# tensorflow/adanet

Hardware: NVIDIA H100
Metric: candidate-train examples/sec per AdaNet iteration (higher is better)
Workload: dtype f32

## Files before the change

### adanet_b200/_lib.py

```python

from __future__ import annotations

import ctypes
import os
from ctypes import POINTER, c_char_p, c_float, c_int, c_int64, c_void_p

_HERE = os.path.dirname(os.path.abspath(__file__))
LIB_PATH = os.path.join(_HERE, "csrc", "libadanet_b200.so")

ACT_NONE, ACT_RELU = 0, 1
HEAD_SOFTMAX_XENT, HEAD_MSE, HEAD_SIGMOID_XENT = 0, 1, 2
MIX_SCALAR, MIX_VECTOR, MIX_MATRIX = 0, 1, 2
OPT_SGD, OPT_MOMENTUM, OPT_RMSPROP, OPT_ADAM, OPT_MOMENTUM_COSINE = 0, 1, 2, 3, 4
PATH_AUTO, PATH_SIMT, PATH_TCGEN05 = 0, 1, 2
PLANES_TF32, PLANES_F16 = 0, 1
(Q_VERSION, Q_DENSE_BWD_WS, Q_HEAD_WS, Q_DENSE_FWD_PATH, Q_SM_COUNT, Q_LAUNCH_COUNT, Q_DENSE_BWD_PATH,
 Q_DENSE_FWD_WS, Q_PLANES_BYTES, Q_DENSE_BWD_P_WS, Q_COLSUM_WS, Q_CONV_STEM_BWD_WS, Q_PLANE_FORMAT,
 Q_TMA_MAP_CACHE_HITS, Q_TMA_MAP_CACHE_MISSES) = range(15)

EXPORTS = (
    "adn_last_error", "adn_init", "adn_query", "adn_set_dense_path", "adn_dense_fwd", "adn_dense_bwd", "adn_head_loss",
    "adn_ensemble_head", "adn_opt_step", "adn_l1_norm", "adn_ema_update", "adn_record_scalars",
    "adn_counter_add", "adn_planes_split", "adn_planes_merge", "adn_dense_fwd_p", "adn_dense_bwd_p", "adn_colsum",
    "adn_opt_step_p", "adn_head_loss_p", "adn_dense_fwd_p_group", "adn_dense_bwd_p_group",
    "adn_l1_grad_add", "adn_conv_stem_fwd", "adn_conv_stem_bwd", "adn_set_plane_format", "adn_plane_overflow",
    "adn_planes_split_scaled", "adn_head_group", "adn_head_bookkeeping", "adn_opt_step_group",
)


class FwdOp(ctypes.Structure):
  _fields_ = [("xp", c_void_p), ("wp", c_void_p), ("bias", c_void_p), ("yp", c_void_p), ("y", c_void_p),
              ("in_", c_int64), ("out", c_int64), ("act", ctypes.c_int32), ("reserved", ctypes.c_int32),
              ("dropout_rate", c_float), ("dropout_seed", ctypes.c_uint32), ("dropout_layer", ctypes.c_int32),
              ("reserved2", ctypes.c_int32), ("dropout_step_dev", c_void_p)]


class BwdOp(ctypes.Structure):
  _fields_ = [("xp", c_void_p), ("wp", c_void_p), ("dzp", c_void_p), ("dxp", c_void_p), ("dx", c_void_p),
              ("dx_colsum", c_void_p), ("dw", c_void_p), ("in_", c_int64), ("out", c_int64),
              ("x_relu_mask", ctypes.c_int32), ("dz_log2_scale", ctypes.c_int32), ("workspace", c_void_p),
              ("workspace_bytes", c_int64), ("dx_mul", c_float), ("reserved2", c_float)]


class HeadOp(ctypes.Structure):
  _fields_ = [("head", ctypes.c_int32), ("mixture_type", ctypes.c_int32), ("members_host", POINTER(c_void_p)),
              ("n_members", ctypes.c_int32), ("reg_is_zero", ctypes.c_int32), ("w", c_void_p), ("bias", c_void_p),
              ("gammas_host", POINTER(c_float)), ("reg_multiplier", c_float), ("dz_log2_scale", ctypes.c_int32),
              ("labels", c_void_p), ("labels_f", c_void_p), ("out3", c_void_p), ("dw", c_void_p), ("dbias", c_void_p),
              ("dens", c_void_p), ("ens_out", c_void_p), ("dens_planes", c_void_p), ("colsum_only", ctypes.c_int32),
# ... 128 lines not shown
```

### adanet_b200/core/engine.py

```python

from __future__ import annotations

import ctypes
import math
from dataclasses import dataclass, field
from typing import Dict, List, Optional, Sequence, Tuple

import numpy as np
import torch

from adanet_b200 import _lib

_HEAD_KIND = {"softmax_xent": _lib.HEAD_SOFTMAX_XENT, "mse": _lib.HEAD_MSE, "sigmoid_xent": _lib.HEAD_SIGMOID_XENT}
_MIX_KIND = {"scalar": _lib.MIX_SCALAR, "vector": _lib.MIX_VECTOR, "matrix": _lib.MIX_MATRIX}
_OPT_KIND = {"sgd": _lib.OPT_SGD, "momentum": _lib.OPT_MOMENTUM, "rmsprop": _lib.OPT_RMSPROP, "adam": _lib.OPT_ADAM,
             "momentum_cosine": _lib.OPT_MOMENTUM_COSINE}
_OPT_DEFAULTS = {"sgd": (), "momentum": (), "rmsprop": (0.9, 0.0, 1e-10), "adam": (0.9, 0.999, 1e-8),
                 "momentum_cosine": (0.0,)}
TRACE_FIELDS = ("sub_loss", "ens_loss", "adanet_loss", "ema")
EVAL_METRICS = ("adanet_loss", "loss", "average_loss", "accuracy")


def accuracy_of(logits: torch.Tensor, labels: torch.Tensor) -> float:
  if logits.shape[1] > 1:
# ... 215 lines not shown
      self.stem_k = torch.as_tensor(k).to(device)
      self.stem_b = torch.as_tensor(np.ascontiguousarray(bs[0], dtype=np.float32)).to(device)
      self.stem_out = new_planes(batch, dims[0], device)
      self.stem_arg = torch.zeros((batch * dims[0] // 16,), dtype=torch.int32, device=device)
      ws, bs = ws[1:], bs[1:]
    self.in_dim = int(np.prod(self.image_shape)) if self.stem else self.dims[0]
    self.fmt = _lib.plane_format()
    assert len(ws) == len(dims) - 1
    self.ws = [torch.as_tensor(np.ascontiguousarray(w, dtype=np.float32)).to(device) for w in ws]
    self.bs = [torch.as_tensor(np.ascontiguousarray(b, dtype=np.float32)).to(device) for b in bs]
    for i, w in enumerate(self.ws):
      if tuple(w.shape) != (dims[i], dims[i + 1]):
        raise ValueError("kernel %d of %s has shape %s, want %s" % (i, name, tuple(w.shape), (dims[i], dims[i + 1])))
    self.planes = planes_enabled()
    n = len(self.ws)
    if self.planes:
      self.acts = [None] * (n - 1) + [torch.empty((batch, dims[-1]), dtype=torch.float32, device=device)]
      self.hp = [new_planes(batch, d, device) for d in dims[1:-1]]
      self.wps = [new_planes(dims[i], dims[i + 1], device) for i in range(n)]
      self.refresh_planes()
      self.fwd_ws_bytes, self.fwd_ws = 0, None
    else:
      self.acts = [torch.empty((batch, d), dtype=torch.float32, device=device) for d in dims[1:]]
      self.hp, self.wps = None, None
      fwd_ws = max(_lib.query(_lib.Q_DENSE_FWD_WS, batch, dims[i], dims[i + 1]) for i in range(n))
      self.fwd_ws_bytes = fwd_ws
      self.fwd_ws = torch.empty((max(fwd_ws, 16),), dtype=torch.uint8, device=device)

  def ensure_format(self):
    if not self.planes or self.fmt == _lib.plane_format():
      return
    self.fmt = _lib.plane_format()
    n = len(self.ws)
    self.hp = [new_planes(self.batch, d, self.device) for d in self.dims[1:-1]]
    self.wps = [new_planes(self.dims[i], self.dims[i + 1], self.device) for i in range(n)]
    if self.stem:
# ... 37 lines not shown
    out = torch.empty((self.batch, self.dims[-2]), dtype=torch.float32, device=self.device)
    _lib.check(_lib.load().adn_planes_merge(self.hp[-1].data_ptr(), self.batch, self.dims[-2], out.data_ptr(),
                                            torch.cuda.current_stream(self.device).cuda_stream), "adn_planes_merge")
    return out

  def fwd_op(self, i: int, xp: torch.Tensor, step_dev: Optional[torch.Tensor] = None) -> "_lib.FwdOp":
    last = i == len(self.ws) - 1
    src = (self.stem_out if self.stem else xp) if i == 0 else self.hp[i - 1]
    op = _lib.FwdOp(src.data_ptr(), self.wps[i].data_ptr(), self.bs[i].data_ptr(),
                    None if last else self.hp[i].data_ptr(), self.acts[i].data_ptr() if last else None,
                    self.dims[i], self.dims[i + 1], _lib.ACT_NONE if last else _lib.ACT_RELU, 0)
    d = self.dropout[i] if (self.dropout and step_dev is not None and not last and i < len(self.dropout)) else None
    if d is not None:
      op.dropout_rate, op.dropout_seed, op.dropout_layer = float(d[0]), int(d[1]) & 0xffffffff, i
      op.dropout_step_dev = step_dev.data_ptr()
    return op

  def dx_mul(self, i: int) -> float:
    d = self.dropout[i] if (self.dropout and 0 <= i < len(self.dropout)) else None
    return 1.0 / (1.0 - float(d[0])) if d is not None else 1.0

  def forward(self, lib, x: torch.Tensor, sp: int, xp: Optional[torch.Tensor] = None):
    n = len(self.ws)
    if self.planes:
      hp = xp
      if self.stem:
        self.stem_forward(lib, x, sp)
        hp = self.stem_out
      for i in range(n):
        last = i == n - 1
# ... 555 lines not shown
    st["pending"] = False

  def _enqueue_waves(self):
    lib = self.lib
    main = torch.cuda.current_stream(self.device)
    sp = main.cuda_stream
    bag = [c for c in self.candidates if c.bagged]
    if bag:
      for c in bag:
        if c.xp_own is not None:
          _lib.check(lib.adn_planes_split(c.x_own.data_ptr(), self.batch, c.net.in_dim, c.xp_own.data_ptr(), sp),
                     "adn_planes_split")
        else:
          c.net.stem_forward(lib, c.x_own, sp)
      for w in range(max(len(c.net.ws) for c in bag)):
        ops = [c.net.fwd_op(w, c.xp_own, self.step_dev) for c in bag if w < len(c.net.ws)]
        _lib.check(lib.adn_dense_fwd_p_group((_lib.FwdOp * len(ops))(*ops), len(ops), self.batch, sp),
                   "adn_dense_fwd_p_group")
      for c in bag:
        lab_i = c.labels_own if self.labels is not None else None
        lab_f = c.labels_own if self.labels is None else None
        c.enqueue_sub_loss(lab_i, lab_f, sp, loss_out=c.own_loss)
      for k in range(max(len(c.net.ws) for c in bag)):
        ops = [c.bwd_op(k, c.xp_own) for c in bag if k < len(c.net.ws)]
        _lib.check(lib.adn_dense_bwd_p_group((_lib.BwdOp * len(ops))(*ops), len(ops), self.batch, sp),
                   "adn_dense_bwd_p_group")
      for c in bag:
        if c.net.stem:
          c.enqueue_stem_bwd(c.x_own, sp)
        c.enqueue_sub_update(sp)
    self._split_x(sp)
# ... 1 lines not shown
      if c.xp_local is not None:
        _lib.check(lib.adn_planes_split(self.x.data_ptr() + c.row0 * self.in_dim * 4, c.batch, self.in_dim,
                                        c.xp_local.data_ptr(), sp), "adn_planes_split")
    xp_of = lambda c: c.xp_local if c.xp_local is not None else self.xp
    x_of = lambda c: self.x[c.row0:c.row0 + c.batch] if c.comm is not None else self.x
    for f in self.frozen:
      if f.stem:
        f.stem_forward(lib, self.x, sp)
    for c in self.candidates:
      if c.net.stem:
        c.net.stem_forward(lib, x_of(c), sp)
    fwd = ([(f, self.xp, self.batch, None) for f in self.frozen] +
           [(c.net, xp_of(c), c.batch, self.step_dev) for c in self.candidates])
    for w in range(max(len(n.ws) for n, _, _, _ in fwd)):
      for bsz in sorted({b for _, _, b, _ in fwd}, reverse=True):
        ops = [n.fwd_op(w, xp, sd) for n, xp, b, sd in fwd if b == bsz and w < len(n.ws)]
        if ops:
          _lib.check(lib.adn_dense_fwd_p_group((_lib.FwdOp * len(ops))(*ops), len(ops), bsz, sp), "adn_dense_fwd_p_group")
    hops = [(c.sub_head_op(self.labels, self.labels_f), c.batch) for c in self.candidates]
    hops += [(h.head_op(self.labels, self.labels_f), h.batch) for _, h, _ in self.heads if h.groupable]
    for bsz in sorted({b for _, b in hops}, reverse=True):
      ops = [o for o, b in hops if b == bsz]
      _lib.check(lib.adn_head_group((_lib.HeadOp * len(ops))(*ops), len(ops), bsz, self.C, sp), "adn_head_group")
    for _, h, _ in self.heads:
      if not h.groupable:
        h.enqueue(self.labels, self.labels_f, self.step_dev, sp, self.xp, bookkeeping=False)
    trained = [c for c in self.candidates if not c.bagged]
    for k in range(max([len(c.net.ws) for c in trained] or [0])):
      for bsz in sorted({c.batch for c in trained}, reverse=True):
        ops = [c.bwd_op(k, xp_of(c)) for c in trained if c.batch == bsz and k < len(c.net.ws)]
        if ops:
# ... 234 lines not shown
```

### adanet_b200/csrc/api.cu

```cuda
#include <stdarg.h>
#include <stdlib.h>
#include <string.h>

#include "common.cuh"
#include "dense_simt.cuh"
#include "dense_tc.cuh"
#include "planes.cuh"

namespace adn {
namespace conv { int64_t bwd_workspace_bytes(int64_t batch, int cin, int f); int init(); }
namespace convtc { int init(); }

thread_local char g_err[512] = "";
std::atomic<long long> g_launches{0};
static std::atomic<int> g_path{ADN_PATH_AUTO};
static std::atomic<int> g_sm_count{0};

int fail(int code, const char* fmt, ...) {
  va_list ap;
  va_start(ap, fmt);
  vsnprintf(g_err, sizeof(g_err), fmt, ap);
  va_end(ap);
  return code;
}
// ... 81 lines not shown
      int64_t t = tc::dense_bwd_workspace_bytes(a, b, c);
      *out_host = s > t ? s : t;
      return ADN_OK;
    }
    case ADN_Q_DENSE_FWD_WORKSPACE_BYTES:
      *out_host = (pick_fwd_path(a, b, c) == ADN_PATH_TCGEN05) ? tc::dense_fwd_workspace_bytes(a, b, c) : 0;
      return ADN_OK;
    case ADN_Q_HEAD_WORKSPACE_BYTES: *out_host = head_workspace_bytes_public(a, b, c) + 256; return ADN_OK;
    case ADN_Q_DENSE_FWD_PATH: *out_host = pick_fwd_path(a, b, c); return ADN_OK;
    case ADN_Q_DENSE_BWD_PATH: *out_host = pick_bwd_path(a, b, c); return ADN_OK;
    case ADN_Q_SM_COUNT: *out_host = sm_count(); return ADN_OK;
    case ADN_Q_PLANES_BYTES: *out_host = pl::planes_bytes(pl::format(), a, b); return ADN_OK;
    case ADN_Q_PLANE_FORMAT: *out_host = pl::format(); return ADN_OK;
    case ADN_Q_TMA_MAP_CACHE_HITS: *out_host = pl::map_cache_hits(); return ADN_OK;
    case ADN_Q_TMA_MAP_CACHE_MISSES: *out_host = pl::map_cache_misses(); return ADN_OK;
    case ADN_Q_DENSE_BWD_P_WORKSPACE_BYTES: *out_host = pl::dense_bwd_workspace_bytes(a, b, c); return ADN_OK;
    case ADN_Q_COLSUM_WORKSPACE_BYTES: *out_host = 64 * b * (int64_t)sizeof(float) + 256; return ADN_OK;
    case ADN_Q_CONV_STEM_BWD_WORKSPACE_BYTES: *out_host = conv::bwd_workspace_bytes(a, (int)b, (int)c); return ADN_OK;
    case ADN_Q_LAUNCH_COUNT: *out_host = g_launches.load(); return ADN_OK;
    default: return fail(ADN_ERR_INVALID, "adn_query: unknown key %d", key);
  }
}

extern "C" int adn_dense_fwd(const float* x, const float* w, const float* b, float* y, int64_t batch, int64_t in,
                             int64_t out, int act, void* workspace, int64_t workspace_bytes, void* stream) {
  if (!x || !w || !y) return fail(ADN_ERR_INVALID, "adn_dense_fwd: null pointer");
  if (batch <= 0 || in <= 0 || out <= 0 || batch > INT32_MAX || in > INT32_MAX || out > INT32_MAX)
    return fail(ADN_ERR_INVALID, "adn_dense_fwd: bad shape [%lld,%lld]x[%lld,%lld]", (long long)batch,
                (long long)in, (long long)in, (long long)out);
  if (act != ADN_ACT_NONE && act != ADN_ACT_RELU) return fail(ADN_ERR_INVALID, "adn_dense_fwd: bad act %d", act);
// ... 92 lines not shown
    if (!ops[i].xp || !ops[i].wp) return fail(ADN_ERR_INVALID, "adn_dense_fwd_p_group: op %d: null pointer", i);
    if ((ops[i].yp == nullptr) == (ops[i].y == nullptr))
      return fail(ADN_ERR_INVALID, "adn_dense_fwd_p_group: op %d: exactly one of yp / y", i);
    if (bad_shape(batch, ops[i].in, ops[i].out)) return fail(ADN_ERR_INVALID, "adn_dense_fwd_p_group: op %d: bad shape", i);
    if (ops[i].act != ADN_ACT_NONE && ops[i].act != ADN_ACT_RELU)
      return fail(ADN_ERR_INVALID, "adn_dense_fwd_p_group: op %d: bad act %d", i, ops[i].act);
    o[i] = pl::FwdOp{ops[i].xp, ops[i].wp, ops[i].bias, ops[i].yp, ops[i].y, ops[i].in, ops[i].out, ops[i].act};
    if (ops[i].dropout_rate != 0.f) {
      if (!(ops[i].dropout_rate > 0.f && ops[i].dropout_rate < 1.f) || !ops[i].yp || !ops[i].dropout_step_dev)
        return fail(ADN_ERR_INVALID, "adn_dense_fwd_p_group: op %d: dropout needs 0 < rate < 1, planes out and a step counter", i);
      o[i].dropout_rate = ops[i].dropout_rate;
      o[i].dropout_seed = ops[i].dropout_seed;
      o[i].dropout_layer = ops[i].dropout_layer;
      o[i].dropout_step = ops[i].dropout_step_dev;
    }
  }
  return pl::dense_fwd_group(pl::format(), o, n, batch, as_stream(stream));
}

extern "C" int adn_dense_bwd_p_group(const adn_bwd_op* ops, int n, int64_t batch, void* stream) {
  if (n < 0 || (n > 0 && !ops)) return fail(ADN_ERR_INVALID, "adn_dense_bwd_p_group: bad ops");
  if (n > 256) return fail(ADN_ERR_UNSUPPORTED, "adn_dense_bwd_p_group: n %d > 256", n);
  pl::BwdOp o[256];
  for (int i = 0; i < n; ++i) {
    const adn_bwd_op& p = ops[i];
    if (!p.xp || !p.dzp || !p.workspace) return fail(ADN_ERR_INVALID, "adn_dense_bwd_p_group: op %d: null pointer", i);
    if ((p.dxp || p.dx) && !p.wp) return fail(ADN_ERR_INVALID, "adn_dense_bwd_p_group: op %d: wp required for dx", i);
    if (p.dxp && p.dx) return fail(ADN_ERR_INVALID, "adn_dense_bwd_p_group: op %d: at most one of dxp / dx", i);
    if (p.dx_colsum && !(p.dxp || p.dx)) return fail(ADN_ERR_INVALID, "adn_dense_bwd_p_group: op %d: dx_colsum needs dx", i);
    if (bad_shape(batch, p.in, p.out)) return fail(ADN_ERR_INVALID, "adn_dense_bwd_p_group: op %d: bad shape", i);
// ... 9 lines not shown
```

### adanet_b200/csrc/planes.cu

```cuda
#include <cuda.h>
#include <cudaTypedefs.h>

#include <stdlib.h>
#include <string.h>

#include <algorithm>
#include <atomic>
#include <mutex>
#include <string>
#include <unordered_map>
#include <vector>

#include "dense_simt.cuh"
#include "planes.cuh"
#include "wgmma.cuh"

namespace adn {
namespace pl {

static constexpr int BM = 128, BN = 64;
static constexpr int STAGES = 3;
static constexpr int A_TILE = BM * 128;
static constexpr int B_TILE = BN * 128;
static constexpr int STAGE_BYTES = 2 * A_TILE + 2 * B_TILE;
// ... 42 lines not shown
  int ldc;
  int out_nb32;
  int out_tma;
  const float* bias;
  int act;
  uint32_t* out_bits;
  const uint32_t* mask_bits;
  float* colsum_part;
  int colsum_ld;
  float out_mul;
  unsigned int* ovf;
  uint32_t drop_thresh;
  uint32_t drop_key0;
  float drop_scale;
  const int64_t* drop_step;
};

__device__ __forceinline__ uint32_t smem_u32(const void* p) { return (uint32_t)__cvta_generic_to_shared(p); }

__device__ __forceinline__ void mbar_init(uint32_t bar, uint32_t count) {
  asm volatile("mbarrier.init.shared::cta.b64 [%0], %1;" ::"r"(bar), "r"(count));
}
__device__ __forceinline__ void mbar_expect_tx(uint32_t bar, uint32_t bytes) {
  asm volatile("mbarrier.arrive.expect_tx.shared::cta.b64 _, [%0], %1;" ::"r"(bar), "r"(bytes) : "memory");
}
__device__ __forceinline__ void mbar_arrive(uint32_t bar) {
  asm volatile("mbarrier.arrive.shared::cta.b64 _, [%0];" ::"r"(bar) : "memory");
}
__device__ __forceinline__ void mbar_wait(uint32_t bar, uint32_t parity) {
  uint32_t ok = 0;
// ... 21 lines not shown
      : "memory");
}
__device__ __forceinline__ void tma_store_3d(const CUtensorMap* map, uint32_t src, int c0, int c1, int c2) {
  asm volatile("cp.async.bulk.tensor.3d.global.shared::cta.bulk_group [%0, {%2, %3, %4}], [%1];"
               ::"l"(reinterpret_cast<uint64_t>(map)), "r"(src), "r"(c0), "r"(c1), "r"(c2)
               : "memory");
}
__device__ __forceinline__ void bulk_commit() { asm volatile("cp.async.bulk.commit_group;" ::: "memory"); }
__device__ __forceinline__ void bulk_wait_read0() { asm volatile("cp.async.bulk.wait_group.read 0;" ::: "memory"); }
__device__ __forceinline__ void bulk_wait_read1() { asm volatile("cp.async.bulk.wait_group.read 1;" ::: "memory"); }
__device__ __forceinline__ void bulk_wait0() { asm volatile("cp.async.bulk.wait_group 0;" ::: "memory"); }
__device__ __forceinline__ void fence_async_smem() { asm volatile("fence.proxy.async.shared::cta;" ::: "memory"); }
__device__ __forceinline__ void sts_v4(uint32_t addr, uint32_t a, uint32_t b, uint32_t c, uint32_t d) {
  asm volatile("st.shared.v4.b32 [%0], {%1, %2, %3, %4};" ::"r"(addr), "r"(a), "r"(b), "r"(c), "r"(d) : "memory");
}
__device__ __forceinline__ void tma_prefetch_desc(const CUtensorMap* map) {
  asm volatile("prefetch.tensormap [%0];" ::"l"(reinterpret_cast<uint64_t>(map)) : "memory");
}

struct Item {
  int m0, n0, kb0, nkb, split;
};
__device__ __forceinline__ int fast_div(int n, float inv) { return (int)(((float)n + 0.5f) * inv); }

__device__ __forceinline__ Item decode_item(const GemmParams& g, int item) {
  Item it;
  it.split = (g.splits == 1) ? 0 : fast_div(item, g.inv_tiles);
  const int t = item - it.split * g.tiles;
  if (g.m_fastest) {
    const int tn = fast_div(t, g.inv_tiles_m);
// ... 28 lines not shown
#pragma unroll
    for (int q = 0; q < 16; ++q) {
      const __half2 h2 = __floats2half2_rn(a[2 * q], a[2 * q + 1]);
      const float2 hf = __half22float2(h2);
      const __half2 l2 = __floats2half2_rn((a[2 * q] - hf.x) * 2048.0f, (a[2 * q + 1] - hf.y) * 2048.0f);
      hw[q] = *reinterpret_cast<const uint32_t*>(&h2);
      lw[q] = *reinterpret_cast<const uint32_t*>(&l2);
    }
    __half* hp = reinterpret_cast<__half*>(g.out) + poff;
    __half* lp = reinterpret_cast<__half*>(g.out_lo) + poff;
    st_global_v8(hp, reinterpret_cast<const uint32_t(&)[8]>(hw[0]));
    st_global_v8(hp + 16, reinterpret_cast<const uint32_t(&)[8]>(hw[8]));
    st_global_v8(lp, reinterpret_cast<const uint32_t(&)[8]>(lw[0]));
    st_global_v8(lp + 16, reinterpret_cast<const uint32_t(&)[8]>(lw[8]));
  } else {
    uint32_t hw[32], lw[32];
#pragma unroll
    for (int j = 0; j < 32; ++j) {
      float h, l;
      split_tf32(a[j], h, l);
      hw[j] = __float_as_uint(h);
      lw[j] = __float_as_uint(l);
    }
    float* hp = reinterpret_cast<float*>(g.out) + poff;
    float* lp = reinterpret_cast<float*>(g.out_lo) + poff;
#pragma unroll
    for (int q = 0; q < 4; ++q) {
      st_global_v8(hp + 8 * q, reinterpret_cast<const uint32_t(&)[8]>(hw[8 * q]));
      st_global_v8(lp + 8 * q, reinterpret_cast<const uint32_t(&)[8]>(lw[8 * q]));
    }
  }
}

__device__ __forceinline__ void store_slice_tma(const CUtensorMap* o_hi, const CUtensorMap* o_lo, uint32_t slab_hi,
                                                uint32_t slab_lo, const float* a, int lane, int mrow0, int cbase) {
  uint32_t w[16], lw[16];
#pragma unroll
  for (int q = 0; q < 16; ++q) {
    const __half2 h2 = __floats2half2_rn(a[2 * q], a[2 * q + 1]);
    const float2 hf = __half22float2(h2);
    const __half2 l2 = __floats2half2_rn((a[2 * q] - hf.x) * 2048.0f, (a[2 * q + 1] - hf.y) * 2048.0f);
    w[q] = *reinterpret_cast<const uint32_t*>(&h2);
    lw[q] = *reinterpret_cast<const uint32_t*>(&l2);
  }
// ... 8 lines not shown
    tma_store_3d(o_hi, slab_hi, cbase & 63, mrow0, cbase >> 6);
    bulk_commit();
    bulk_wait_read1();
  }
  __syncwarp();
#pragma unroll
  for (uint32_t j = 0; j < 4; ++j) sts_v4(slab_lo + roff + ((j ^ sw) << 4), lw[4 * j], lw[4 * j + 1], lw[4 * j + 2], lw[4 * j + 3]);
  fence_async_smem();
  __syncwarp();
  if (lane == 0) {
    tma_store_3d(o_lo, slab_lo, cbase & 63, mrow0, cbase >> 6);
    bulk_commit();
  }
}

template <int FMT>
__device__ __forceinline__ void emit_slice_fwd_planes(const GemmParams& g, float* a, uint32_t drop_step, int lane, int mrow0,
                                                      int cbase, const CUtensorMap* o_hi, const CUtensorMap* o_lo,
                                                      uint32_t slab_hi, uint32_t slab_lo) {
  const int my_row = mrow0 + lane;
  const int kbo = cbase >> 5;
  if (kbo >= g.out_nb32) return;
  const uint32_t cmask = (cbase + 32 <= g.N) ? 0xffffffffu : ((cbase < g.N) ? ((1u << (g.N - cbase)) - 1u) : 0u);
  if (g.act == ADN_ACT_RELU) {
#pragma unroll
    for (int j = 0; j < 32; ++j) a[j] = fmaxf(a[j], 0.f);
  }
  if (g.drop_thresh != 0u) {
    const uint32_t key = g.drop_key0 + drop_step * 0xC2B2AE3Du;
    const uint32_t base = (uint32_t)my_row * (uint32_t)g.N + (uint32_t)cbase;
#pragma unroll
    for (int j = 0; j < 32; ++j) {
      uint32_t x = (base + (uint32_t)j) ^ key;
      x ^= x >> 16; x *= 0x7feb352du; x ^= x >> 15; x *= 0x846ca68bu; x ^= x >> 16;
      a[j] = (x >= g.drop_thresh) ? a[j] * g.drop_scale : 0.f;
    }
  }
  if (cmask != 0xffffffffu) {
#pragma unroll
    for (int j = 0; j < 32; ++j)
      if (!((cmask >> j) & 1u)) a[j] = 0.f;
  }
  if (FMT == FMT_F16 && g.out_tma) store_slice_tma(o_hi, o_lo, slab_hi, slab_lo, a, lane, mrow0, cbase);
  else if (my_row < g.M) store_row32_planes<FMT>(g, a, my_row, cbase);
  uint32_t bits = 0u;
#pragma unroll
  for (int j = 0; j < 32; ++j) bits |= (a[j] > 0.f) ? (1u << j) : 0u;
  if (my_row < g.M) g.out_bits[(size_t)kbo * g.M + my_row] = bits;
}

template <int W>
__device__ __forceinline__ void colsum_round(float* a, int lane) {
  const bool upper = (lane & W) != 0;
#pragma unroll
  for (int j = 0; j < W; ++j) {
    const float x = a[j], y = a[j + W];
    const float mine = upper ? y : x;
    const float send = upper ? x : y;
    a[j] = mine + __shfl_xor_sync(0xffffffffu, send, W);
  }
}

// ... 22 lines not shown
    colsum_round<8>(a, lane);
    colsum_round<4>(a, lane);
    colsum_round<2>(a, lane);
    colsum_round<1>(a, lane);
    const int col = cbase + lane;
    if (col < g.colsum_ld) g.colsum_part[(size_t)(mrow0 >> 5) * g.colsum_ld + col] = a[0];
  }
}

template <int FMT, int EPI>
__device__ __forceinline__ void emit_slice(const GemmParams& g, const bool OUT_PLANES, float* a, uint32_t mwq, float* stage,
                                           int lane, int mrow0, int cbase, int rows_ok, float* dense, bool dense_vec,
                                           const bool bias_in_acc = false, const CUtensorMap* o_hi = nullptr,
                                           const CUtensorMap* o_lo = nullptr, uint32_t drop_step = 0u) {
  if (EPI == EPI_BIAS_ACT && OUT_PLANES && bias_in_acc) {
    emit_slice_fwd_planes<FMT>(g, a, drop_step, lane, mrow0, cbase, o_hi, o_lo, smem_u32(stage),
                               smem_u32(stage + EPI_STAGE_FLOATS));
    return;
  }
  if (EPI == EPI_MASK && OUT_PLANES && bias_in_acc) {
    emit_slice_mask_planes<FMT>(g, a, mwq, lane, mrow0, cbase, o_hi, o_lo, smem_u32(stage), smem_u32(stage + EPI_STAGE_FLOATS));
    return;
  }
  constexpr int SW = 16;
  constexpr int CH = SW / 4;
  constexpr int RPI = 32 / CH;
  const int cc = lane % CH;
  const int rsub = lane / CH;
  const int my_row = mrow0 + lane;
  const int kbo = cbase >> 5;
  const bool live = (OUT_PLANES ? (kbo < g.out_nb32) : (cbase < g.N)) && rows_ok > 0;
  const uint32_t cmask = (cbase + 32 <= g.N) ? 0xffffffffu : ((cbase < g.N) ? ((1u << (g.N - cbase)) - 1u) : 0u);
// ... 154 lines not shown
template <int EPI>
__device__ __forceinline__ EpiItem epi_fetch(const Group& grp, int& cur, int& next0, int item, int tile_row) {
  EpiItem e;
  cur = find_problem(grp, cur, item, next0);
  e.p = cur;
  const GemmParams& g = grp.p[cur].g;
  e.it = decode_item(g, item - grp.p[cur].item0);
  e.mw0 = e.mw1 = 0xffffffffu;
  if (EPI == EPI_MASK && g.mask_bits) {
    const int my_row = e.it.m0 + tile_row, kbo = e.it.n0 >> 5;
    const bool row_ok = my_row < g.M;
    e.mw0 = (row_ok && kbo < g.out_nb32) ? __ldg(g.mask_bits + (size_t)kbo * g.M + my_row) : 0u;
    e.mw1 = (row_ok && kbo + 1 < g.out_nb32) ? __ldg(g.mask_bits + (size_t)(kbo + 1) * g.M + my_row) : 0u;
  }
  e.drop_step = (EPI == EPI_BIAS_ACT && g.drop_thresh != 0u) ? (uint32_t)(*g.drop_step) : 0u;
  return e;
}

template <int R> __device__ __forceinline__ void setmaxnreg_inc() { asm volatile("setmaxnreg.inc.sync.aligned.u32 %0;" ::"n"(R)); }
template <int R> __device__ __forceinline__ void setmaxnreg_dec() { asm volatile("setmaxnreg.dec.sync.aligned.u32 %0;" ::"n"(R)); }

__device__ __forceinline__ int acc_off(int row, int col) {
  return row * BN + ((((col >> 2) ^ row) & 7) | ((col >> 2) & 8)) * 4 + (col & 3);
}

template <int FMT>
__device__ __forceinline__ void fold_chunk(float (&acc)[32], const float (&H)[32], const float (&S)[32]) {
#pragma unroll
  for (int j = 0; j < 32; ++j) acc[j] += H[j];
  if (FMT == FMT_F16) {
// ... 142 lines not shown
    for (int item = blockIdx.x; item < n_items; item += gridDim.x, ++tcount) {
      const EpiItem e = nx;
      if (item + (int)gridDim.x < n_items) nx = epi_fetch<EPI>(grp, cur, next0, item + gridDim.x, row);
      const GemmParams& g = grp.p[e.p].g;
      const Item& it = e.it;
      const uint32_t buf = tcount & 1u;
      mbar_wait(smem_u32(&tile_full[buf]), (tcount >> 1) & 1u);
      const float* tile = acc_stage + buf * ACC_TILE_FLOATS;
      const int mrow0 = it.m0 + 32 * ew;
      float* dense = reinterpret_cast<float*>(g.out);
      if (EPI == EPI_PARTIAL) dense += (size_t)it.split * g.M * g.N;
      const bool out_planes = g.out_planes != 0;
      const bool dense_vec = !out_planes && ((g.ldc & 3) == 0) && ((reinterpret_cast<uintptr_t>(dense) & 15) == 0);
      const int rows_ok = min(32, g.M - mrow0);
      const uint32_t mw0 = e.mw0, mw1 = e.mw1;
#pragma unroll 1
      for (int h = 0; h < 2; ++h) {
        const int cs = 32 * h;
        float acc[32];
#pragma unroll
        for (int q = 0; q < 8; ++q) {
          const float4 v = *reinterpret_cast<const float4*>(tile + acc_off(row, cs + 4 * q));
          acc[4 * q] = v.x; acc[4 * q + 1] = v.y; acc[4 * q + 2] = v.z; acc[4 * q + 3] = v.w;
        }
        if (h == 1) mbar_arrive(smem_u32(&tile_empty[buf]));
        const int ncol0 = it.n0 + cs;
        const uint32_t mw = h ? mw1 : mw0;
        if (FMT == FMT_F16 && !out_planes) {
          if (lane == 0) bulk_wait_read0();
          __syncwarp();
        }
        emit_slice<FMT, EPI>(g, out_planes, acc, mw, stage, lane, mrow0, ncol0, rows_ok, dense, dense_vec, true,
                             &grp.p[e.p].o_hi, &grp.p[e.p].o_lo, e.drop_step);
      }
    }
    if (FMT == FMT_F16 && lane == 0) bulk_wait0();
    return;
  }

// ... 406 lines not shown

static int max_dw_splits(int64_t in, int64_t out) {
  int64_t s = (16LL << 20) / std::max<int64_t>(1, in * out);
  if (s > MAX_SPLITS) s = MAX_SPLITS;
  if (s < 1) s = 1;
  return (int)s;
}

int64_t dense_bwd_workspace_bytes(int64_t batch, int64_t in, int64_t out) {
  int64_t b = align_up((int64_t)max_dw_splits(in, out) * in * out * (int64_t)sizeof(float), 256);
  b += align_up(ceil_div(batch, 32) * in * (int64_t)sizeof(float), 256);
  b += align_up(64 * in * (int64_t)sizeof(float), 256);
  return b + 512;
}

int dense_fwd_group(int fmt, const FwdOp* ops, int n, int64_t batch, cudaStream_t st) {
  if (n <= 0) return ADN_OK;
  const int bk = fmt_bk(fmt);
  std::vector<GemmDesc> d((size_t)n);
  for (int i = 0; i < n; ++i) {
    const FwdOp& o = ops[i];
    GemmDesc& e = d[(size_t)i];
    e.a = operand(fmt, o.xp, batch, o.in, 0);
    e.b = operand(fmt, o.wp, o.in, o.out, 1);
    GemmParams g{};
    g.M = (int)batch; g.N = (int)o.out;
    g.total_kb = (int)ceil_div(o.in, bk); g.kb_per_split = g.total_kb; g.splits = 1;
    g.bias = o.bias; g.act = o.act;
    g.out_mul = 1.0f;
    if (o.dropout_rate > 0.f) {
      if (!o.yp || !o.dropout_step) return fail(ADN_ERR_INVALID, "pl dense_fwd: dropout needs planes out and a step counter");
      const double t = (double)o.dropout_rate * 4294967296.0;
      g.drop_thresh = t >= 4294967295.0 ? 0xffffffffu : (uint32_t)t;
      if (g.drop_thresh == 0u) g.drop_thresh = 1u;
      g.drop_key0 = o.dropout_seed * 0x9E3779B1u + (uint32_t)o.dropout_layer * 0x85EBCA77u + 0x27D4EB2Fu;
      g.drop_scale = 1.0f / (1.0f - o.dropout_rate);
      g.drop_step = o.dropout_step;
    }
    if (o.yp) {
      const PlaneView v = plane_view(fmt, o.yp, batch, o.out);
      g.out_planes = 1;
      g.out = v.hi; g.out_lo = v.lo; g.out_nb32 = (int)bits_blocks(fmt, o.out);
      g.out_bits = v.bits;
    } else {
      g.out = o.y; g.ldc = (int)o.out;
    }
    e.g = g;
  }
  return launch_group<EPI_BIAS_ACT>(fmt, d.data(), n, st, "pl dense_fwd gemm");
}

int dense_bwd_group(int fmt, const BwdOp* ops, int n, int64_t batch, cudaStream_t st) {
  if (n <= 0) return ADN_OK;
  const int bk = fmt_bk(fmt);
  const int workers = sm_count();
  struct Carve { float* part; float* cspart; float* cspart2; int splits; };
  std::vector<Carve> cv((size_t)n);
  std::vector<GemmDesc> dwd, dxd;
  const int64_t kb_b = ceil_div(batch, bk);
  int64_t best_kps = kb_b;
  {
    static std::mutex mu;
    static std::unordered_map<std::string, int64_t> memo;
    std::string key = std::to_string(batch) + ":" + std::to_string(fmt);
// ... 135 lines not shown
```

### adanet_b200/csrc/planes.cuh

```cuda
#pragma once
#include "common.cuh"
#include "plane_fmt.cuh"

namespace adn {
namespace pl {

int init();
int set_format(int fmt);
int read_overflow(int* out_host, int reset, cudaStream_t st);
long long map_cache_hits();
long long map_cache_misses();
int64_t dense_bwd_workspace_bytes(int64_t batch, int64_t in, int64_t out);

int split(int fmt, const float* src, int64_t rows, int64_t cols, void* planes, int log2_scale, cudaStream_t st);
int merge(int fmt, const void* planes, int64_t rows, int64_t cols, float* dst, cudaStream_t st);
struct FwdOp {
  const void* xp;
  const void* wp;
  const float* bias;
  void* yp;
  float* y;
  int64_t in, out;
  int act;
  float dropout_rate = 0.f;
  uint32_t dropout_seed = 0;
  int dropout_layer = 0;
  const int64_t* dropout_step = nullptr;
};
struct BwdOp {
  const void* xp;
  const void* wp;
  const void* dzp;
  void* dxp;
  float* dx;
  float* dx_colsum;
  float* dw;
  int64_t in, out;
  int x_relu_mask;
  int dz_log2_scale;
  void* ws;
  int64_t ws_bytes;
  float dx_mul = 1.f;
};
// ... 11 lines not shown
```

### include/adanet_b200.h

```cpp
#ifndef ADANET_B200_H_
#define ADANET_B200_H_

#include <stdint.h>

#ifdef __cplusplus
extern "C" {
#endif

#define ADN_OK 0
#define ADN_ERR_INVALID (-22)
#define ADN_ERR_CUDA (-5)
#define ADN_ERR_UNSUPPORTED (-95)
#define ADN_ERR_WORKSPACE (-12)

#define ADN_ACT_NONE 0
#define ADN_ACT_RELU 1

#define ADN_HEAD_SOFTMAX_XENT 0
#define ADN_HEAD_MSE 1
#define ADN_HEAD_SIGMOID_XENT 2

#define ADN_MIX_SCALAR 0
#define ADN_MIX_VECTOR 1
#define ADN_MIX_MATRIX 2
// ... 14 lines not shown
#define ADN_Q_VERSION 0
#define ADN_Q_DENSE_BWD_WORKSPACE_BYTES 1
#define ADN_Q_HEAD_WORKSPACE_BYTES 2
#define ADN_Q_DENSE_FWD_PATH 3
#define ADN_Q_SM_COUNT 4
#define ADN_Q_LAUNCH_COUNT 5
#define ADN_Q_DENSE_BWD_PATH 6
#define ADN_Q_DENSE_FWD_WORKSPACE_BYTES 7
#define ADN_Q_PLANES_BYTES 8
#define ADN_Q_DENSE_BWD_P_WORKSPACE_BYTES 9
#define ADN_Q_COLSUM_WORKSPACE_BYTES 10
#define ADN_Q_CONV_STEM_BWD_WORKSPACE_BYTES 11
#define ADN_Q_PLANE_FORMAT 12
#define ADN_Q_TMA_MAP_CACHE_HITS 13
#define ADN_Q_TMA_MAP_CACHE_MISSES 14

const char* adn_last_error(void);
int adn_init(void);
int adn_query(int key, int64_t a, int64_t b, int64_t c, int64_t* out_host);
int adn_set_dense_path(int path);
int adn_set_plane_format(int fmt);
int adn_plane_overflow(int* flag_host, int reset, void* stream);

int adn_dense_fwd(const float* x, const float* w, const float* b, float* y,
                  int64_t batch, int64_t in, int64_t out, int act,
                  void* workspace, int64_t workspace_bytes, void* stream);

int adn_dense_bwd(const float* x, const float* w, const float* dz,
                  float* dx, float* dw, float* db,
                  int64_t batch, int64_t in, int64_t out, int x_relu_mask,
// ... 23 lines not shown
                    int x_relu_mask, int dz_log2_scale, void* workspace, int64_t workspace_bytes, void* stream);
typedef struct adn_fwd_op {
  const void* xp;
  const void* wp;
  const float* bias;
  void* yp;
  float* y;
  int64_t in, out;
  int32_t act;
  int32_t reserved;
  float dropout_rate;
  uint32_t dropout_seed;
  int32_t dropout_layer;
  int32_t reserved2;
  const int64_t* dropout_step_dev;
} adn_fwd_op;
typedef struct adn_bwd_op {
  const void* xp;
  const void* wp;
  const void* dzp;
  void* dxp;
  float* dx;
  float* dx_colsum;
  float* dw;
  int64_t in, out;
  int32_t x_relu_mask;
  int32_t dz_log2_scale;
  void* workspace;
  int64_t workspace_bytes;
  float dx_mul;
// ... 88 lines not shown
```

Baseline: 9.401 million.

## Fuse small-width logits layer into the preceding dense forward GEMM epilogue

When the final layer has at most 16 output columns, its matmul is computed inside the epilogue of the penultimate planes GEMM. Each column tile writes per-row partial logits to a workspace, and a grouped reduce kernel sums the partials into the logits buffer. This removes the separate last-layer GEMM launch and the re-read of the hidden activations, at the cost of a heavier epilogue, extra register pressure and an added reduction pass. The change also splits the TF32 store loop into smaller chunks and switches shared-memory accumulator loads to explicit vector loads.

```diff
diff --git a/adanet_b200/_lib.py b/adanet_b200/_lib.py
--- a/adanet_b200/_lib.py
+++ b/adanet_b200/_lib.py
@@ -16,7 +16,8 @@
 PLANES_TF32, PLANES_F16 = 0, 1
 (Q_VERSION, Q_DENSE_BWD_WS, Q_HEAD_WS, Q_DENSE_FWD_PATH, Q_SM_COUNT, Q_LAUNCH_COUNT, Q_DENSE_BWD_PATH,
  Q_DENSE_FWD_WS, Q_PLANES_BYTES, Q_DENSE_BWD_P_WS, Q_COLSUM_WS, Q_CONV_STEM_BWD_WS, Q_PLANE_FORMAT,
- Q_TMA_MAP_CACHE_HITS, Q_TMA_MAP_CACHE_MISSES) = range(15)
+ Q_TMA_MAP_CACHE_HITS, Q_TMA_MAP_CACHE_MISSES, Q_FWD_NEXT_WS) = range(16)
+FWD_NEXT_MAX_C = 16
 
 EXPORTS = (
     "adn_last_error", "adn_init", "adn_query", "adn_set_dense_path", "adn_dense_fwd", "adn_dense_bwd", "adn_head_loss",
@@ -32,7 +33,9 @@
   _fields_ = [("xp", c_void_p), ("wp", c_void_p), ("bias", c_void_p), ("yp", c_void_p), ("y", c_void_p),
               ("in_", c_int64), ("out", c_int64), ("act", ctypes.c_int32), ("reserved", ctypes.c_int32),
               ("dropout_rate", c_float), ("dropout_seed", ctypes.c_uint32), ("dropout_layer", ctypes.c_int32),
-              ("reserved2", ctypes.c_int32), ("dropout_step_dev", c_void_p)]
+              ("reserved2", ctypes.c_int32), ("dropout_step_dev", c_void_p),
+              ("next_w", c_void_p), ("next_bias", c_void_p), ("next_y", c_void_p), ("next_c", c_int64),
+              ("next_ws", c_void_p), ("next_ws_bytes", c_int64)]
 
 
 class BwdOp(ctypes.Structure):
diff --git a/adanet_b200/core/engine.py b/adanet_b200/core/engine.py
--- a/adanet_b200/core/engine.py
+++ b/adanet_b200/core/engine.py
@@ -253,12 +253,17 @@
         raise ValueError("kernel %d of %s has shape %s, want %s" % (i, name, tuple(w.shape), (dims[i], dims[i + 1])))
     self.planes = planes_enabled()
     n = len(self.ws)
+    self.fuse_logits = False
     if self.planes:
       self.acts = [None] * (n - 1) + [torch.empty((batch, dims[-1]), dtype=torch.float32, device=device)]
       self.hp = [new_planes(batch, d, device) for d in dims[1:-1]]
       self.wps = [new_planes(dims[i], dims[i + 1], device) for i in range(n)]
       self.refresh_planes()
       self.fwd_ws_bytes, self.fwd_ws = 0, None
+      self.fuse_logits = n >= 2 and dims[-1] <= _lib.FWD_NEXT_MAX_C
+      if self.fuse_logits:
+        self.fuse_ws_bytes = _lib.query(_lib.Q_FWD_NEXT_WS, batch, dims[-2], dims[-1])
+        self.fuse_ws = torch.empty((self.fuse_ws_bytes // 4,), dtype=torch.float32, device=device)
     else:
       self.acts = [torch.empty((batch, d), dtype=torch.float32, device=device) for d in dims[1:]]
       self.hp, self.wps = None, None
@@ -326,6 +331,17 @@
     if d is not None:
       op.dropout_rate, op.dropout_seed, op.dropout_layer = float(d[0]), int(d[1]) & 0xffffffff, i
       op.dropout_step_dev = step_dev.data_ptr()
+    return op
+
+  def fwd_wave_op(self, i: int, xp: torch.Tensor, step_dev: Optional[torch.Tensor] = None) -> Optional["_lib.FwdOp"]:
+    n = len(self.ws)
+    if not self.fuse_logits or i < n - 2:
+      return self.fwd_op(i, xp, step_dev)
+    if i == n - 1:
+      return None
+    op = self.fwd_op(i, xp, step_dev)
+    op.next_w, op.next_bias, op.next_y = self.ws[-1].data_ptr(), self.bs[-1].data_ptr(), self.acts[-1].data_ptr()
+    op.next_c, op.next_ws, op.next_ws_bytes = self.dims[-1], self.fuse_ws.data_ptr(), self.fuse_ws_bytes
     return op
 
   def dx_mul(self, i: int) -> float:
@@ -911,7 +927,10 @@
         else:
           c.net.stem_forward(lib, c.x_own, sp)
       for w in range(max(len(c.net.ws) for c in bag)):
-        ops = [c.net.fwd_op(w, c.xp_own, self.step_dev) for c in bag if w < len(c.net.ws)]
+        ops = [c.net.fwd_wave_op(w, c.xp_own, self.step_dev) for c in bag if w < len(c.net.ws)]
+        ops = [o for o in ops if o is not None]
+        if not ops:
+          continue
         _lib.check(lib.adn_dense_fwd_p_group((_lib.FwdOp * len(ops))(*ops), len(ops), self.batch, sp),
                    "adn_dense_fwd_p_group")
       for c in bag:
@@ -943,7 +962,8 @@
            [(c.net, xp_of(c), c.batch, self.step_dev) for c in self.candidates])
     for w in range(max(len(n.ws) for n, _, _, _ in fwd)):
       for bsz in sorted({b for _, _, b, _ in fwd}, reverse=True):
-        ops = [n.fwd_op(w, xp, sd) for n, xp, b, sd in fwd if b == bsz and w < len(n.ws)]
+        ops = [n.fwd_wave_op(w, xp, sd) for n, xp, b, sd in fwd if b == bsz and w < len(n.ws)]
+        ops = [o for o in ops if o is not None]
         if ops:
           _lib.check(lib.adn_dense_fwd_p_group((_lib.FwdOp * len(ops))(*ops), len(ops), bsz, sp), "adn_dense_fwd_p_group")
     hops = [(c.sub_head_op(self.labels, self.labels_f), c.batch) for c in self.candidates]
diff --git a/adanet_b200/csrc/api.cu b/adanet_b200/csrc/api.cu
--- a/adanet_b200/csrc/api.cu
+++ b/adanet_b200/csrc/api.cu
@@ -119,6 +119,7 @@
     case ADN_Q_PLANE_FORMAT: *out_host = pl::format(); return ADN_OK;
     case ADN_Q_TMA_MAP_CACHE_HITS: *out_host = pl::map_cache_hits(); return ADN_OK;
     case ADN_Q_TMA_MAP_CACHE_MISSES: *out_host = pl::map_cache_misses(); return ADN_OK;
+    case ADN_Q_FWD_NEXT_WORKSPACE_BYTES: *out_host = pl::fwd_next_workspace_bytes(a, b, c); return ADN_OK;
     case ADN_Q_DENSE_BWD_P_WORKSPACE_BYTES: *out_host = pl::dense_bwd_workspace_bytes(a, b, c); return ADN_OK;
     case ADN_Q_COLSUM_WORKSPACE_BYTES: *out_host = 64 * b * (int64_t)sizeof(float) + 256; return ADN_OK;
     case ADN_Q_CONV_STEM_BWD_WORKSPACE_BYTES: *out_host = conv::bwd_workspace_bytes(a, (int)b, (int)c); return ADN_OK;
@@ -241,6 +242,12 @@
       o[i].dropout_layer = ops[i].dropout_layer;
       o[i].dropout_step = ops[i].dropout_step_dev;
     }
+    o[i].next_w = ops[i].next_w;
+    o[i].next_bias = ops[i].next_bias;
+    o[i].next_y = ops[i].next_y;
+    o[i].next_c = ops[i].next_c;
+    o[i].next_ws = ops[i].next_ws;
+    o[i].next_ws_bytes = ops[i].next_ws_bytes;
   }
   return pl::dense_fwd_group(pl::format(), o, n, batch, as_stream(stream));
 }
diff --git a/adanet_b200/csrc/planes.cu b/adanet_b200/csrc/planes.cu
--- a/adanet_b200/csrc/planes.cu
+++ b/adanet_b200/csrc/planes.cu
@@ -80,6 +80,10 @@
   uint32_t drop_key0;
   float drop_scale;
   const int64_t* drop_step;
+  const float* fuse_w;
+  const float* fuse_bias;
+  float* fuse_part;
+  int fuse_c;
 };
 
 __device__ __forceinline__ uint32_t smem_u32(const void* p) { return (uint32_t)__cvta_generic_to_shared(p); }
@@ -131,6 +135,9 @@
 __device__ __forceinline__ void sts_v4(uint32_t addr, uint32_t a, uint32_t b, uint32_t c, uint32_t d) {
   asm volatile("st.shared.v4.b32 [%0], {%1, %2, %3, %4};" ::"r"(addr), "r"(a), "r"(b), "r"(c), "r"(d) : "memory");
 }
+__device__ __forceinline__ void lds_v4(uint32_t addr, float& a, float& b, float& c, float& d) {
+  asm volatile("ld.shared.v4.f32 {%0, %1, %2, %3}, [%4];" : "=f"(a), "=f"(b), "=f"(c), "=f"(d) : "r"(addr) : "memory");
+}
 __device__ __forceinline__ void tma_prefetch_desc(const CUtensorMap* map) {
   asm volatile("prefetch.tensormap [%0];" ::"l"(reinterpret_cast<uint64_t>(map)) : "memory");
 }
@@ -189,20 +196,20 @@
     st_global_v8(lp, reinterpret_cast<const uint32_t(&)[8]>(lw[0]));
     st_global_v8(lp + 16, reinterpret_cast<const uint32_t(&)[8]>(lw[8]));
   } else {
-    uint32_t hw[32], lw[32];
-#pragma unroll
-    for (int j = 0; j < 32; ++j) {
-      float h, l;
-      split_tf32(a[j], h, l);
-      hw[j] = __float_as_uint(h);
-      lw[j] = __float_as_uint(l);
-    }
     float* hp = reinterpret_cast<float*>(g.out) + poff;
     float* lp = reinterpret_cast<float*>(g.out_lo) + poff;
 #pragma unroll
     for (int q = 0; q < 4; ++q) {
-      st_global_v8(hp + 8 * q, reinterpret_cast<const uint32_t(&)[8]>(hw[8 * q]));
-      st_global_v8(lp + 8 * q, reinterpret_cast<const uint32_t(&)[8]>(lw[8 * q]));
+      uint32_t hw[8], lw[8];
+#pragma unroll
+      for (int j = 0; j < 8; ++j) {
+        float h, l;
+        split_tf32(a[8 * q + j], h, l);
+        hw[j] = __float_as_uint(h);
+        lw[j] = __float_as_uint(l);
+      }
+      st_global_v8(hp + 8 * q, hw);
+      st_global_v8(lp + 8 * q, lw);
     }
   }
 }
@@ -241,10 +248,56 @@
   }
 }
 
-template <int FMT>
+static constexpr int FUSE_QB = 8;
+__device__ __forceinline__ void sts_f32(uint32_t addr, float v) {
+  asm volatile("st.shared.f32 [%0], %1;" ::"r"(addr), "f"(v) : "memory");
+}
+__device__ __forceinline__ float lds_f32(uint32_t addr) {
+  float v;
+  asm volatile("ld.shared.f32 %0, [%1];" : "=f"(v) : "r"(addr) : "memory");
+  return v;
+}
+template <int C>
+__device__ __forceinline__ void fuse_next_slice(const float* __restrict__ w, int nrows, const float* a, float* p,
+                                                uint32_t slabs, int lane) {
+  if (nrows >= 32) {
+    const float4* w4 = reinterpret_cast<const float4*>(w);
+    static_assert((8 * C) % FUSE_QB == 0, "whole load batches");
+#pragma unroll
+    for (int q0 = 0; q0 < 8 * C; q0 += FUSE_QB) {
+      float4 t[FUSE_QB];
+#pragma unroll
+      for (int b = 0; b < FUSE_QB; ++b) t[b] = __ldg(w4 + q0 + b);
+#pragma unroll
+      for (int b = 0; b < FUSE_QB; ++b) {
+        const float tv[4] = {t[b].x, t[b].y, t[b].z, t[b].w};
+#pragma unroll
+        for (int v = 0; v < 4; ++v) {
+          const int f = 4 * (q0 + b) + v;
+          p[f % C] = fmaf(a[f / C], tv[v], p[f % C]);
+        }
+      }
+    }
+  } else if (nrows > 0) {
+    if (lane == 0) bulk_wait_read0();
+    __syncwarp();
+#pragma unroll
+    for (int j = 0; j < 32; ++j) sts_f32(slabs + (uint32_t)(j * 32 + lane) * 4u, a[j]);
+    __syncwarp();
+#pragma unroll 1
+    for (int j = 0; j < nrows; ++j) {
+      const float aj = lds_f32(slabs + (uint32_t)(j * 32 + lane) * 4u);
+#pragma unroll
+      for (int c = 0; c < C; ++c) p[c] = fmaf(aj, __ldg(w + j * C + c), p[c]);
+    }
+    __syncwarp();
+  }
+}
+
+template <int FMT, bool FUSE>
 __device__ __forceinline__ void emit_slice_fwd_planes(const GemmParams& g, float* a, uint32_t drop_step, int lane, int mrow0,
                                                       int cbase, const CUtensorMap* o_hi, const CUtensorMap* o_lo,
-                                                      uint32_t slab_hi, uint32_t slab_lo) {
+                                                      uint32_t slab_hi, uint32_t slab_lo, float* fp) {
   const int my_row = mrow0 + lane;
   const int kbo = cbase >> 5;
   if (kbo >= g.out_nb32) return;
@@ -268,11 +321,24 @@
     for (int j = 0; j < 32; ++j)
       if (!((cmask >> j) & 1u)) a[j] = 0.f;
   }
+  uint32_t bits = 0u;
+#pragma unroll
+  for (int j = 0; j < 32; ++j) bits |= (a[j] > 0.f) ? (1u << j) : 0u;
+  if (FUSE) {
+    const float* w = g.fuse_w + (size_t)cbase * g.fuse_c;
+    const int nrows = g.N - cbase;
+    switch (g.fuse_c) {
+#define ADN_FUSE_CASE(CC) case CC: fuse_next_slice<CC>(w, nrows, a, fp, slab_hi, lane); break;
+      ADN_FUSE_CASE(1) ADN_FUSE_CASE(2) ADN_FUSE_CASE(3) ADN_FUSE_CASE(4)
+      ADN_FUSE_CASE(5) ADN_FUSE_CASE(6) ADN_FUSE_CASE(7) ADN_FUSE_CASE(8)
+      ADN_FUSE_CASE(9) ADN_FUSE_CASE(10) ADN_FUSE_CASE(11) ADN_FUSE_CASE(12)
+      ADN_FUSE_CASE(13) ADN_FUSE_CASE(14) ADN_FUSE_CASE(15) ADN_FUSE_CASE(16)
+#undef ADN_FUSE_CASE
+      default: break;
+    }
+  }
   if (FMT == FMT_F16 && g.out_tma) store_slice_tma(o_hi, o_lo, slab_hi, slab_lo, a, lane, mrow0, cbase);
   else if (my_row < g.M) store_row32_planes<FMT>(g, a, my_row, cbase);
-  uint32_t bits = 0u;
-#pragma unroll
-  for (int j = 0; j < 32; ++j) bits |= (a[j] > 0.f) ? (1u << j) : 0u;
   if (my_row < g.M) g.out_bits[(size_t)kbo * g.M + my_row] = bits;
 }
 
@@ -325,8 +391,8 @@
                                            const bool bias_in_acc = false, const CUtensorMap* o_hi = nullptr,
                                            const CUtensorMap* o_lo = nullptr, uint32_t drop_step = 0u) {
   if (EPI == EPI_BIAS_ACT && OUT_PLANES && bias_in_acc) {
-    emit_slice_fwd_planes<FMT>(g, a, drop_step, lane, mrow0, cbase, o_hi, o_lo, smem_u32(stage),
-                               smem_u32(stage + EPI_STAGE_FLOATS));
+    emit_slice_fwd_planes<FMT, false>(g, a, drop_step, lane, mrow0, cbase, o_hi, o_lo, smem_u32(stage),
+                                      smem_u32(stage + EPI_STAGE_FLOATS), nullptr);
     return;
   }
   if (EPI == EPI_MASK && OUT_PLANES && bias_in_acc) {
@@ -511,6 +577,13 @@
     e.mw1 = (row_ok && kbo + 1 < g.out_nb32) ? __ldg(g.mask_bits + (size_t)(kbo + 1) * g.M + my_row) : 0u;
   }
   e.drop_step = (EPI == EPI_BIAS_ACT && g.drop_thresh != 0u) ? (uint32_t)(*g.drop_step) : 0u;
+  if (EPI == EPI_BIAS_ACT && g.fuse_c != 0 && tile_row < 32) {
+    const int floats = min(BN, g.N - e.it.n0) * g.fuse_c;
+    if (32 * tile_row < floats) {
+      const float* line = g.fuse_w + (size_t)e.it.n0 * g.fuse_c + 32 * tile_row;
+      asm volatile("prefetch.global.L1 [%0];" ::"l"(line));
+    }
+  }
   return e;
 }
 
@@ -683,15 +756,37 @@
       const bool dense_vec = !out_planes && ((g.ldc & 3) == 0) && ((reinterpret_cast<uintptr_t>(dense) & 15) == 0);
       const int rows_ok = min(32, g.M - mrow0);
       const uint32_t mw0 = e.mw0, mw1 = e.mw1;
+      if (EPI == EPI_BIAS_ACT && g.fuse_c != 0) {
+        const int fuse_c = g.fuse_c;
+        float fp[ADN_FWD_NEXT_MAX_C];
+#pragma unroll
+        for (int c = 0; c < ADN_FWD_NEXT_MAX_C; ++c)
+          fp[c] = (c < fuse_c && it.n0 == 0 && g.fuse_bias) ? __ldg(g.fuse_bias + c) : 0.f;
+#pragma unroll 1
+        for (int h = 0; h < 2; ++h) {
+          float acc[32];
+#pragma unroll
+          for (int q = 0; q < 8; ++q)
+            lds_v4(smem_u32(tile + acc_off(row, 32 * h + 4 * q)), acc[4 * q], acc[4 * q + 1], acc[4 * q + 2], acc[4 * q + 3]);
+          if (h == 1) mbar_arrive(smem_u32(&tile_empty[buf]));
+          emit_slice_fwd_planes<FMT, true>(g, acc, e.drop_step, lane, mrow0, it.n0 + 32 * h, &grp.p[e.p].o_hi, &grp.p[e.p].o_lo,
+                                     smem_u32(stage), smem_u32(stage + EPI_STAGE_FLOATS), fp);
+        }
+        if (it.m0 + row < g.M) {
+          float* dst = g.fuse_part + ((size_t)(it.n0 / BN) * g.M + (it.m0 + row)) * fuse_c;
+#pragma unroll
+          for (int c = 0; c < ADN_FWD_NEXT_MAX_C; ++c)
+            if (c < fuse_c) dst[c] = fp[c];
+        }
+        continue;
+      }
 #pragma unroll 1
       for (int h = 0; h < 2; ++h) {
         const int cs = 32 * h;
         float acc[32];
 #pragma unroll
-        for (int q = 0; q < 8; ++q) {
-          const float4 v = *reinterpret_cast<const float4*>(tile + acc_off(row, cs + 4 * q));
-          acc[4 * q] = v.x; acc[4 * q + 1] = v.y; acc[4 * q + 2] = v.z; acc[4 * q + 3] = v.w;
-        }
+        for (int q = 0; q < 8; ++q)
+          lds_v4(smem_u32(tile + acc_off(row, cs + 4 * q)), acc[4 * q], acc[4 * q + 1], acc[4 * q + 2], acc[4 * q + 3]);
         if (h == 1) mbar_arrive(smem_u32(&tile_empty[buf]));
         const int ncol0 = it.n0 + cs;
         const uint32_t mw = h ? mw1 : mw0;
@@ -1128,10 +1223,31 @@
   return b + 512;
 }
 
+int64_t fwd_next_workspace_bytes(int64_t batch, int64_t out, int64_t next_c) {
+  return ceil_div(out, (int64_t)BN) * batch * next_c * (int64_t)sizeof(float);
+}
+
 int dense_fwd_group(int fmt, const FwdOp* ops, int n, int64_t batch, cudaStream_t st) {
   if (n <= 0) return ADN_OK;
   const int bk = fmt_bk(fmt);
+  for (int i = 0; i < n; ++i) {
+    const FwdOp& o = ops[i];
+    if (o.next_c == 0 && !o.next_w && !o.next_bias && !o.next_y && !o.next_ws) continue;
+    if (o.next_c < 1 || o.next_c > ADN_FWD_NEXT_MAX_C)
+      return fail(ADN_ERR_UNSUPPORTED, "pl dense_fwd: op %d: next_c %lld outside [1, %d]", i, (long long)o.next_c,
+                  ADN_FWD_NEXT_MAX_C);
+    if (!o.yp || !o.next_w || !o.next_y || !o.next_ws)
+      return fail(ADN_ERR_INVALID, "pl dense_fwd: op %d: a fused next layer needs planes out, next_w, next_y and next_ws", i);
+    if ((reinterpret_cast<uintptr_t>(o.next_w) & 15) || ((reinterpret_cast<uintptr_t>(o.next_ws) |
+         reinterpret_cast<uintptr_t>(o.next_y) | reinterpret_cast<uintptr_t>(o.next_bias)) & 3))
+      return fail(ADN_ERR_INVALID, "pl dense_fwd: op %d: next_w must be 16 B aligned, next_bias / next_y / next_ws 4 B", i);
+    const int64_t need = fwd_next_workspace_bytes(batch, o.out, o.next_c);
+    if (o.next_ws_bytes < need)
+      return fail(ADN_ERR_WORKSPACE, "pl dense_fwd: op %d: next_ws %lld < %lld bytes", i, (long long)o.next_ws_bytes,
+                  (long long)need);
+  }
   std::vector<GemmDesc> d((size_t)n);
+  std::vector<simt::ReduceJob> jobs;
   for (int i = 0; i < n; ++i) {
     const FwdOp& o = ops[i];
     GemmDesc& e = d[(size_t)i];
@@ -1159,9 +1275,17 @@
     } else {
       g.out = o.y; g.ldc = (int)o.out;
     }
+    if (o.next_c) {
+      g.fuse_w = o.next_w; g.fuse_bias = o.next_bias; g.fuse_c = (int)o.next_c;
+      g.fuse_part = reinterpret_cast<float*>(o.next_ws);
+      const int64_t n_y = batch * o.next_c;
+      jobs.push_back(simt::ReduceJob{g.fuse_part, o.next_y, n_y, (int)ceil_div(o.out, (int64_t)BN), n_y, 1.0f});
+    }
     e.g = g;
   }
-  return launch_group<EPI_BIAS_ACT>(fmt, d.data(), n, st, "pl dense_fwd gemm");
+  int rc = launch_group<EPI_BIAS_ACT>(fmt, d.data(), n, st, "pl dense_fwd gemm");
+  if (rc) return rc;
+  return simt::reduce_partials_group(jobs.data(), (int)jobs.size(), st);
 }
 
 int dense_bwd_group(int fmt, const BwdOp* ops, int n, int64_t batch, cudaStream_t st) {
diff --git a/adanet_b200/csrc/planes.cuh b/adanet_b200/csrc/planes.cuh
--- a/adanet_b200/csrc/planes.cuh
+++ b/adanet_b200/csrc/planes.cuh
@@ -26,7 +26,14 @@
   uint32_t dropout_seed = 0;
   int dropout_layer = 0;
   const int64_t* dropout_step = nullptr;
+  const float* next_w = nullptr;
+  const float* next_bias = nullptr;
+  float* next_y = nullptr;
+  int64_t next_c = 0;
+  void* next_ws = nullptr;
+  int64_t next_ws_bytes = 0;
 };
+int64_t fwd_next_workspace_bytes(int64_t batch, int64_t out, int64_t next_c);
 struct BwdOp {
   const void* xp;
   const void* wp;
diff --git a/include/adanet_b200.h b/include/adanet_b200.h
--- a/include/adanet_b200.h
+++ b/include/adanet_b200.h
@@ -52,6 +52,9 @@
 #define ADN_Q_PLANE_FORMAT 12
 #define ADN_Q_TMA_MAP_CACHE_HITS 13
 #define ADN_Q_TMA_MAP_CACHE_MISSES 14
+#define ADN_Q_FWD_NEXT_WORKSPACE_BYTES 15
+
+#define ADN_FWD_NEXT_MAX_C 16
 
 const char* adn_last_error(void);
 int adn_init(void);
@@ -105,6 +108,12 @@
   int32_t dropout_layer;
   int32_t reserved2;
   const int64_t* dropout_step_dev;
+  const float* next_w;
+  const float* next_bias;
+  float* next_y;
+  int64_t next_c;
+  void* next_ws;
+  int64_t next_ws_bytes;
 } adn_fwd_op;
 typedef struct adn_bwd_op {
   const void* xp;
```

After: 9.133 million, median of 6. -2.9%, worse.
